# iden3/circom

Measured on NVIDIA H100. Metric: witnesses/s, higher is better.
Workload: dtype u256 (8x u32 limbs, Montgomery)

## Files before the change

### __graft_entry__.py

```python
from __future__ import annotations

import os
import sys

ROOT = os.path.dirname(os.path.abspath(__file__))
if ROOT not in sys.path:
    sys.path.insert(0, ROOT)


def build() -> None:
    from circom_b200 import build as b
    b.build()
    import circom_b200
    from circom_b200 import native
    from tests.util import build_hostsim
    build_hostsim()
    from oracle import build_ref, build_calcs, c_oracle
    c_oracle.build()
    if build_ref.have_reference():
        build_ref.build_all()
        build_calcs.build()


def smoke() -> None:
    import random
    from circom_b200.circuit import CircuitDesc
    from circom_b200 import circuits as C
    from circom_b200.witness_calculator import builder, R1cs, limbs_to_ints
    from oracle.ir_eval import evaluate
    d = CircuitDesc("bn128")
    d.set_main(C.all_ops(d))
# ... 18 lines not shown
```

### circom_b200/csrc/capi.cu

```cuda
#include <cuda_runtime.h>
#include <dlfcn.h>
#include <emmintrin.h>
#include <nccl.h>

#include <cstdio>
#include <cstdlib>
#include <algorithm>
#include <chrono>
#include <condition_variable>
#include <cstring>
#include <functional>
#include <map>
#include <tuple>
#include <memory>
#include <mutex>
#include <thread>
#include <stdexcept>
#include <string>
#include <vector>

#include "../../include/circom_b200.h"
#include <cub/device/device_radix_sort.cuh>

#include "kernels.cuh"
// ... 248 lines not shown
    if ((rc = upload(&d.input_slot, t.input_slot.data(), t.input_slot.size() * 4))) return rc;
    if ((rc = upload(&d.fn_code, t.fn_code.data(), t.fn_code.size() * 4))) return rc;
    if ((rc = upload(&d.fn_info, t.fn_info.data(), t.fn_info.size() * 4))) return rc;
    if ((rc = upload(&d.call_tab, t.call_tab.data(), t.call_tab.size() * 4))) return rc;
    if ((rc = upload(&d.wloc, t.witness_slot.data(), t.witness_slot.size() * 4))) return rc;
    if ((rc = upload(&d.pk_bit, L.bit_loc.data(), L.bit_loc.size() * 4))) return rc;
    if ((rc = upload(&d.pk_u64, L.u64_loc.data(), L.u64_loc.size() * 4))) return rc;
    if ((rc = upload(&d.pk_full, L.full_loc.data(), L.full_loc.size() * 4))) return rc;
    c->dev[device] = d;
    out = d;
    return CW_OK;
}

template <int PR, bool CALLS, bool BP, int BT, bool FU>
static void launch_tape_k(const TapeDev &tp, cw_batch *b, u32 tiles, u32 th) {
    constexpr u32 smem = FU ? TAPE_ACC_SMEM : 0u;
    static_assert(TAPE_ACC_SMEM * CW_TAPE_LB <= 48u * 1024u, "the widest CTA stays within the default dynamic shared memory");
    tape_exec_kernel<PR, CALLS, BP, BT, FU><<<tiles, th, smem * th, b->stream>>>(tp, b->slots, b->plane, b->bt_log2,
                                                                                b->first_assert_d, b->err_d, b->batch);
}
template <int PR>
static void launch_tape(const TapeDev &tp, cw_batch *b, u32 tiles, u32 th, bool calls, bool bp, bool fused) {
    if (calls) {
        launch_tape_calls(PR, tp, b->slots, b->plane, b->bt_log2, b->first_assert_d, b->err_d, b->batch, tiles, th, bp, fused,
                          b->stream);
    } else if (fused) {
        if (b->bt_log2 == 5) launch_tape_k<PR, false, true, 5, true>(tp, b, tiles, th);
        else launch_tape_k<PR, false, true, -1, true>(tp, b, tiles, th);
    } else if (bp) {
        if (b->bt_log2 == 0) launch_tape_k<PR, false, true, 0, false>(tp, b, tiles, th);
        else if (b->bt_log2 == 5) launch_tape_k<PR, false, true, 5, false>(tp, b, tiles, th);
        else launch_tape_k<PR, false, true, -1, false>(tp, b, tiles, th);
    } else {
        if (b->bt_log2 == 0) launch_tape_k<PR, false, false, 0, false>(tp, b, tiles, th);
// ... 1956 lines not shown
```

### circom_b200/csrc/flatten.cpp

```cpp
#include <algorithm>
#include <bitset>
#include <cstdio>
#include <cstdlib>
#include <cstring>
#include <functional>
#include <stdexcept>
#include <unordered_map>

#include "../../include/circom_b200.h"
#include "tape.h"

namespace cw {

uint64_t fnv1a(const char *s, size_t n) {
    uint64_t h = 0xCBF29CE484222325ULL;
    for (size_t i = 0; i < n; ++i) {
        h ^= (uint64_t)(int64_t)(signed char)s[i];
        h *= 0x100000001B3ULL;
    }
    return h;
}

namespace {

// ... 1330 lines not shown
            if (!is_assert && !live[n_pre + i]) continue;
            live[n_pre + i] = 1;
            if (o[0] == 45) {
                uint32_t n = pcalls[o[1] + 1];
                for (uint32_t k = 0; k < n; ++k) {
                    uint32_t a = pcalls[o[1] + 2 + k];
                    if (!(a & OPERAND_CONST)) live[a] = 1;
                }
                continue;
            }
            for (int k = 1; k <= 3; ++k) {
                if (k == 3 && c_is_immediate(o[0])) break;
                if (o[k] != NO_SLOT && !(o[k] & OPERAND_CONST)) live[o[k]] = 1;
            }
        }
        constexpr uint32_t FUSE_MAX = 24;
        enum { FR_READER, FR_POSITION, FR_SIZE, FR_CHAIN, FR_N };
        uint64_t refused[FR_N] = {}, refused_op[64] = {};
        std::vector<uint8_t> fusedf(n_prov, 0);
        std::vector<uint32_t> kid_a(n_prov, NO_SLOT), kid_b(n_prov, NO_SLOT);
        {
            std::vector<uint32_t> uses(n_pre + n_prov, 0), cons(n_pre + n_prov, NO_SLOT);
            std::vector<uint8_t> cons_pos(n_pre + n_prov, 0);
            for (size_t i = 0; i < n_prov; ++i) {
                if (!live[n_pre + i]) continue;
                const uint32_t *o = &pops[i * 4];
                if (o[0] == 45) {
                    uint32_t n = pcalls[o[1] + 1];
                    for (uint32_t k = 0; k < n; ++k) {
                        uint32_t x = pcalls[o[1] + 2 + k];
                        if (!(x & OPERAND_CONST)) uses[x] += 2;
                    }
// ... 13 lines not shown
            auto candidate = [&](uint32_t slot, size_t reader, int pos) -> bool {
                if (!fuse_on || slot == NO_SLOT || (slot & OPERAND_CONST) || slot < n_pre) return false;
                const size_t c = slot - n_pre;
                const uint32_t opc = pops[c * 4];
                if (uses[slot] != 1 || cons[slot] != reader || cons_pos[slot] != pos || claimed[slot] >= 0) return false;
                if (is_assert_op(opc) || opc == 45 || opc == 47 || opc == CW_OP_COPY) return false;
                if (opc == CW_OP_INV || opc == CW_OP_POW) return false;
                return true;
            };
            auto decide = [&](size_t i) {
                const uint32_t *o = &pops[i * 4];
                uint32_t ka = candidate(o[1], i, 1) ? o[1] - n_pre : NO_SLOT;
                uint32_t kb = candidate(o[2], i, 2) ? o[2] - n_pre : NO_SLOT;
                if (ka != NO_SLOT && kb != NO_SLOT) {
                    uint32_t deep = need[ka] >= need[kb] ? ka : kb, other = deep == ka ? kb : ka;
                    if (need[other] > 1 || gsize[ka] + gsize[kb] + 1 > FUSE_MAX) {
                        uint32_t drop = gsize[ka] >= gsize[kb] ? kb : ka;
                        if (need[other] > 1) drop = other;
                        ++refused[need[other] > 1 ? FR_CHAIN : FR_SIZE];
                        if (drop == ka) ka = NO_SLOT; else kb = NO_SLOT;
                    }
                }
                if (ka != NO_SLOT && kb == NO_SLOT && gsize[ka] + 1 > FUSE_MAX) { ka = NO_SLOT; ++refused[FR_SIZE]; }
                if (kb != NO_SLOT && ka == NO_SLOT && gsize[kb] + 1 > FUSE_MAX) { kb = NO_SLOT; ++refused[FR_SIZE]; }
                kid_a[i] = ka;
                kid_b[i] = kb;
                uint32_t sz = 1;
                uint8_t nd = 1;
                if (ka != NO_SLOT && kb != NO_SLOT) {
                    sz += gsize[ka] + gsize[kb];
                    nd = (uint8_t)std::max<int>(std::max(need[ka], need[kb]), std::min(need[ka], need[kb]) + 1);
                } else if (ka != NO_SLOT) { sz += gsize[ka]; nd = need[ka]; }
                else if (kb != NO_SLOT) { sz += gsize[kb]; nd = need[kb]; }
                gsize[i] = sz;
// ... 33 lines not shown
                const uint32_t opc = pops[i * 4];
                if (opc == 45 || opc == 47 || opc == CW_OP_INV || opc == CW_OP_POW) continue;
                regroup(i);
                decide(i);
            }
            const char *cenv = getenv("CW_FUSION_CENSUS");
            if (fuse_on && cenv && atoi(cenv)) {
                for (size_t c = 0; c < n_prov; ++c) {
                    const uint32_t s = n_pre + (uint32_t)c, opc = pops[c * 4];
                    if (!live[s] || fusedf[c] || uses[s] != 1 || claimed[s] >= 0 || is_assert_op(opc)) continue;
                    const uint32_t rd = pops[(size_t)cons[s] * 4];
                    if (rd == 45 || rd == 47 || rd == CW_OP_INV || rd == CW_OP_POW) ++refused[FR_READER];
                    else if (cons_pos[s] == 3) ++refused[FR_POSITION];
                    else if (!candidate(s, cons[s], cons_pos[s])) ++refused_op[opc & 63u];
                }
                fprintf(stderr, "fusion census: single-reader values kept in the store: reader INV/POW %llu, operand c %llu, "
                        "FUSE_MAX %llu, chain rule %llu, producer opcode",
                        (unsigned long long)refused[FR_READER], (unsigned long long)refused[FR_POSITION],
                        (unsigned long long)refused[FR_SIZE], (unsigned long long)refused[FR_CHAIN]);
                for (int k = 0; k < 64; ++k)
                    if (refused_op[k]) fprintf(stderr, " %d:%llu", k, (unsigned long long)refused_op[k]);
                fprintf(stderr, "\n");
            }
        }
        std::vector<uint32_t> glevel(n_pre + n_prov, 0);
        std::vector<uint64_t> gsig(n_prov, 0);
        uint32_t max_level = 0;
        size_t n_roots = 0;
        {
            std::vector<uint32_t> ext(n_prov, 0);
            for (size_t i = 0; i < n_prov; ++i) {
                if (!live[n_pre + i]) continue;
                const uint32_t *o = &pops[i * 4];
                uint32_t e = 0;
// ... 46 lines not shown
        }
        for (size_t r = 0; r < order.size(); ++r) {
            uint32_t p = n_pre + order[r];
            if (claimed[p] >= 0) remap[p] = (uint32_t)claimed[p];
            else if (!is_assert_op(pops[(size_t)order[r] * 4])) remap[p] = next_tmp++;
            if (pops[(size_t)order[r] * 4] == 45) {
                const uint32_t *ct = &pcalls[pops[(size_t)order[r] * 4 + 1]];
                const uint32_t *ex = ct + 2 + ct[1];
                for (uint32_t k = 0; k < ex[0]; ++k) {
                    const uint32_t s = ex[1 + k];
                    if (!live[s]) continue;
                    remap[s] = claimed[s] >= 0 ? (uint32_t)claimed[s] : next_tmp++;
                }
            }
        }
        if (next_tmp >= DST_ACC) throw std::runtime_error("circuit too large for the packed tape word (2^24 slots)");
        T.ops.clear();
        T.ops.reserve(n_live_ops(live, n_pre, n_prov) * 4);
        T.items.clear();
        T.items.reserve(n_roots + 1);
        T.level_start.assign(max_level + 1, 0);
        T.n_mul_ops = 0;
        uint32_t prev_level = 0;
        const bool narrow_on = !(flags & (CW_FLAG_NO_NARROW | CW_FLAG_NO_PEEPHOLE));
        auto opd_bits = [&](uint32_t o) -> uint32_t {
            if (o == NO_SLOT) return 0;
            if (o & OPERAND_CONST) return (uint32_t)u256_bitlen(consts[o & 0x7FFFFFFFu]);
            return o < slot_bits.size() ? slot_bits[o] : 256u;
        };
        auto const_amount = [&](uint32_t o, uint32_t &k) {
            if (o == NO_SLOT || !(o & OPERAND_CONST)) return false;
// ... 50 lines not shown
                }
                const uint32_t *ex = &pcalls[o[1] + 2 + n];
                T.call_tab.push_back(ex[0]);
                for (uint32_t k = 0; k < ex[0]; ++k) T.call_tab.push_back(live[ex[1 + k]] ? remap[ex[1 + k]] : NO_SLOT);
                return;
            }
            for (int k = 1; k <= 3; ++k) {
                if (k == 3 && c_is_immediate(o[0])) d[k] = o[k];
                else if (o[k] == NO_SLOT) d[k] = OPERAND_CONST;
                else if (o[k] & OPERAND_CONST) d[k] = o[k];
                else if (k == 1 && acc_a >= 0) d[k] = OPERAND_ACC | (uint32_t)acc_a;
                else if (k == 2 && acc_b >= 0) d[k] = OPERAND_ACC | (uint32_t)acc_b;
                else d[k] = remap[o[k]];
            }
        };
        std::function<void(uint32_t, int)> emit_sub = [&](uint32_t i, int target) {
            const uint32_t ka = kid_a[i], kb = kid_b[i];
            int acc_a = -1, acc_b = -1;
            if (ka != NO_SLOT && kb != NO_SLOT) {
                const bool a_first = subtree_need(ka, kid_a, kid_b) >= subtree_need(kb, kid_a, kid_b);
                if (a_first) { emit_sub(ka, target); emit_sub(kb, target ^ 1); }
                else { emit_sub(kb, target); emit_sub(ka, target ^ 1); }
                acc_a = a_first ? target : (target ^ 1);
                acc_b = a_first ? (target ^ 1) : target;
            } else if (ka != NO_SLOT) { emit_sub(ka, target); acc_a = target; }
            else if (kb != NO_SLOT) { emit_sub(kb, target); acc_b = target; }
            uint32_t d[4];
            word(i, DST_ACC + (uint32_t)target, acc_a, acc_b, d);
            census(i, d[0] & 0xFFu);
            T.ops.insert(T.ops.end(), d, d + 4);
            if (pops[(size_t)i * 4] == CW_OP_MUL) ++T.n_mul_ops;
        };
        for (size_t r = 0; r < order.size(); ++r) {
            const uint32_t i = order[r];
            const uint32_t *o = &pops[(size_t)i * 4];
            const uint32_t lvl = glevel[n_pre + i];
            const uint32_t dst = is_assert_op(o[0]) ? 0u : remap[n_pre + i];
            const uint32_t ka = kid_a[i], kb = kid_b[i];
            const bool single = ka == NO_SLOT && kb == NO_SLOT;
            uint32_t d[4];
            if (single) {
                word(i, dst, -1, -1, d);
                if (o[0] == DOP_BITS && !(flags & CW_FLAG_NO_PEEPHOLE) && lvl == prev_level && !T.ops.empty() &&
// ... 1 lines not shown
                    uint32_t *p = &T.ops[T.ops.size() - 4];
                    if ((p[0] & 0xFFu) == DOP_BITS && p[1] == d[1] && ((p[3] >> 16) & 0xFFu) == 1u && ((d[3] >> 16) & 0xFFu) == 1u) {
                        uint32_t cnt = (p[3] >> 24) + 1u, pk = p[3] & 0xFFFFu, pdst = p[0] >> 8;
                        if (cnt < 32u && (d[3] & 0xFFFFu) == pk + cnt && dst == pdst + cnt) {
                            p[3] += 1u << 24;
                            continue;
                        }
                    }
                }
                if (o[0] != 45) census(i, d[0] & 0xFFu);
                T.items.push_back((uint32_t)(T.ops.size() / 4));
                T.ops.insert(T.ops.end(), d, d + 4);
            } else {
                T.items.push_back((uint32_t)(T.ops.size() / 4));
                int acc_a = -1, acc_b = -1;
                if (ka != NO_SLOT && kb != NO_SLOT) {
                    const bool a_first = subtree_need(ka, kid_a, kid_b) >= subtree_need(kb, kid_a, kid_b);
                    if (a_first) { emit_sub(ka, 0); emit_sub(kb, 1); }
                    else { emit_sub(kb, 0); emit_sub(ka, 1); }
                    acc_a = a_first ? 0 : 1;
                    acc_b = a_first ? 1 : 0;
                } else if (ka != NO_SLOT) { emit_sub(ka, 0); acc_a = 0; }
                else { emit_sub(kb, 0); acc_b = 0; }
                word(i, dst, acc_a, acc_b, d);
                census(i, d[0] & 0xFFu);
                T.ops.insert(T.ops.end(), d, d + 4);
            }
            prev_level = lvl;
            if (o[0] == CW_OP_MUL) ++T.n_mul_ops;
            T.level_start[lvl]++;
        }
        T.items.push_back((uint32_t)(T.ops.size() / 4));
        {
            std::vector<uint32_t> ls(max_level + 1, 0);
            uint32_t acc = 0;
            uint64_t widest = 0;
            for (uint32_t l = 1; l <= max_level; ++l) {
                ls[l - 1] = acc;
// ... 22 lines not shown
                const uint32_t *o = &T.ops[i * 4];
                if ((o[0] & 0xFFu) == DOP_BITS && (o[3] >> 24) && !(o[1] & OPERAND_CONST) && code[o[1]] != NO_SLOT) ok = false;
            }
            for (uint32_t i = 0; ok && i < M.n_in + 1; ++i)
                if (code[remap[i]] != NO_SLOT) ok = false;
            if (next_tmp >= OPERAND_BIT) ok = false;
            if (ok) {
                newid.resize(next_tmp);
                uint32_t nw = 0;
                for (uint32_t s = 0; s < next_tmp; ++s) newid[s] = code[s] == NO_SLOT ? nw++ : code[s];
                uint32_t word = 0;
                for (size_t i = 0; i < n_ops; ++i) {
                    uint32_t *o = &T.ops[i * 4];
                    const uint32_t opc = o[0] & 0xFFu;
                    if (opc == DOP_BITS && (o[3] >> 24)) o[0] = opc | (word++ << 8);
                    else if (!is_assert_op(opc) && (o[0] >> 8) < DST_ACC) o[0] = opc | (newid[o[0] >> 8] << 8);
                    if (opc == 45) continue;
                    for (int k = 1; k <= 3; ++k) {
                        if (k == 3 && c_is_immediate(opc)) break;
                        if (!(o[k] & (OPERAND_CONST | OPERAND_ACC))) o[k] = newid[o[k]];
                    }
                }
                for (size_t i = 0; i < T.call_tab.size();) {
                    const uint32_t n = T.call_tab[i + 1], nx = T.call_tab[i + 2 + n];
                    for (uint32_t k = 0; k < n + 1 + nx; ++k) {
                        if (k == n) continue;
                        uint32_t &e = T.call_tab[i + 2 + k];
                        if (!(e & OPERAND_CONST)) e = newid[e];
                    }
                    i += 3 + n + nx;
                }
// ... 22 lines not shown
                        continue;
                    }
                    for (int k = 1; k <= 3; ++k) {
                        if (k == 3 && c_is_immediate(opc)) break;
                        if (is_tmp(o[k])) last[o[k]] = (uint32_t)l;
                    }
                }
            std::vector<std::vector<uint32_t>> release(n_lv + 1);
            std::vector<uint32_t> free_ids;
            uint32_t next_phys = n_resident;
            for (size_t l = 0; l < n_lv; ++l) {
                for (uint32_t p : release[l]) free_ids.push_back(p);
                for (uint32_t i = T.items[T.level_start[l]]; i < T.items[T.level_start[l + 1]]; ++i) {
                    uint32_t *o = &T.ops[(size_t)i * 4];
                    const uint32_t opc = o[0] & 0xFFu, d = o[0] >> 8;
                    if (is_assert_op(opc) || d >= DST_ACC) continue;
                    const uint32_t run = opc == DOP_BITS ? (o[3] >> 24) + 1u : 1u;
                    if (run > 1) {
                        if (T.n_bitwords || d < n_resident) continue;
                        for (uint32_t j = 0; j < run; ++j) phys[d + j] = next_phys++;
                        continue;
                    }
                    auto alloc = [&](uint32_t d) {
                        if (d < n_resident) return;
                        uint32_t p;
                        if (!free_ids.empty()) { p = free_ids.back(); free_ids.pop_back(); }
                        else p = next_phys++;
                        phys[d] = p;
                        release[std::min<size_t>(std::max<size_t>(last[d], l) + 1, n_lv)].push_back(p);
                    };
                    alloc(d);
                    if (opc == 45) {
                        const uint32_t *ex = &T.call_tab[o[1] + 2 + T.call_tab[o[1] + 1]];
                        for (uint32_t k = 0; k < ex[0]; ++k)
                            if (ex[1 + k] != NO_SLOT) alloc(ex[1 + k]);
                    }
                }
            }
            auto map = [&](uint32_t o) { return is_tmp(o) ? phys[o] : o; };
            for (size_t i = 0; i < n_ops; ++i) {
                uint32_t *o = &T.ops[i * 4];
                const uint32_t opc = o[0] & 0xFFu;
                if (!is_assert_op(opc) && !(opc == DOP_BITS && (o[3] >> 24) && T.n_bitwords) && (o[0] >> 8) >= n_resident &&
                    (o[0] >> 8) < DST_ACC)
                    o[0] = opc | (phys[o[0] >> 8] << 8);
                if (opc == 45) continue;
                for (int k = 1; k <= 3; ++k) {
                    if (k == 3 && c_is_immediate(opc)) break;
                    o[k] = map(o[k]);
                }
            }
            for (size_t i = 0; i < T.call_tab.size();) {
                const uint32_t n = T.call_tab[i + 1], nx = T.call_tab[i + 2 + n];
                for (uint32_t k = 0; k < n + 1 + nx; ++k)
                    if (k != n) T.call_tab[i + 2 + k] = map(T.call_tab[i + 2 + k]);
                i += 3 + n + nx;
            }
            next_tmp = next_phys;
        }
        T.n_resident = n_resident;
        {
            T.n_slot_operands = 0;
            T.n_values = 0;
            T.n_stored = 0;
            const size_t n_ops = T.ops.size() / 4;
            for (size_t i = 0; i < n_ops; ++i) {
                const uint32_t *o = &T.ops[i * 4];
                const uint32_t opc = o[0] & 0xFFu;
                if (!is_assert_op(opc)) T.n_values += opc == DOP_BITS ? (o[3] >> 24) + 1u : 1u;
                if (!is_assert_op(opc) && (o[0] >> 8) < DST_ACC) ++T.n_stored;
                if (opc == 45) {
                    const uint32_t *ex = &T.call_tab[o[1] + 2 + T.call_tab[o[1] + 1]];
                    for (uint32_t k = 0; k < ex[0]; ++k)
                        if (ex[1 + k] != NO_SLOT) { ++T.n_values; ++T.n_stored; }
                    continue;
                }
                for (int k = 1; k <= 3; ++k) {
                    if (k == 3 && c_is_immediate(opc)) break;
                    if (!(o[k] & (OPERAND_CONST | OPERAND_BIT | OPERAND_ACC))) ++T.n_slot_operands;
                }
            }
        }
        T.witness_slot.resize(W);
        for (uint64_t i = 0; i < W; ++i) T.witness_slot[i] = newid.empty() ? (uint32_t)i : newid[i];
        T.input_slot.resize(M.n_in);
// ... 64 lines not shown
    template <class T> void vec(std::vector<T> &v) {
        uint64_t n;
        pod(n);
        if (n > (uint64_t)(end - p) / sizeof(T)) throw std::runtime_error("lowered-circuit blob: bad length");
        v.resize(n);
        if (n) raw(v.data(), n * sizeof(T));
    }
    void str(std::string &s) {
        uint64_t n;
        pod(n);
        if (n > (uint64_t)(end - p)) throw std::runtime_error("lowered-circuit blob: bad length");
        s.assign((const char *)p, n);
        p += n;
    }
};
constexpr uint32_t BLOB_VERSION = 7;
}

void serialize_tape(const Tape &t, std::vector<uint8_t> &out) {
    BlobW w{out};
    w.raw("CB2T", 4);
    w.pod<uint32_t>(BLOB_VERSION);
    w.pod<int32_t>(t.F.prime_id);
    w.pod(t.flags);
    const uint64_t nums[] = {t.n_signals, t.n_witness, t.n_inputs, t.n_outputs, t.n_components, t.n_ir_ops, t.n_mul_ops,
                             t.n_conv_ops, t.max_level_width, t.n_asserts, t.slot_census[0], t.slot_census[1],
                             t.slot_census[2], t.slot_census[3], t.n_slot_operands, t.n_values, t.n_resident, t.n_pre,
                             t.n_slots, t.n_bitwords, t.n_stored};
    w.pod<uint64_t>(sizeof(nums) / 8);
    w.raw(nums, sizeof(nums));
    w.vec(t.ops); w.vec(t.items); w.vec(t.level_start); w.vec(t.consts); w.vec(t.dat_consts); w.vec(t.witness_slot); w.vec(t.input_slot);
    w.vec(t.pk_bit_wire); w.vec(t.pk_u64_wire); w.vec(t.pk_full_wire); w.vec(t.wit_class); w.vec(t.wit_bits);
    w.vec(t.fn_code); w.vec(t.fn_info); w.vec(t.call_tab); w.vec(t.witness2signal);
    w.raw(t.width_census, sizeof(t.width_census));
    w.pod<uint64_t>(t.inputs.size());
    for (const InputInfo &in : t.inputs) {
        w.str(in.name);
        w.pod(in.hash); w.pod(in.signal_id); w.pod(in.size);
    }
    w.vec(t.hashmap);
    const R1csData &r = t.r1cs;
    w.pod<int32_t>(r.prime_id);
    w.pod(r.n_wires); w.pod(r.n_constraints);
// ... 3 lines not shown

void deserialize_tape(const uint8_t *data, size_t len, Tape &t) {
    BlobR r{data, data + len};
    char magic[4];
    r.raw(magic, 4);
    uint32_t ver;
    r.pod(ver);
    if (memcmp(magic, "CB2T", 4) || ver != BLOB_VERSION) throw std::runtime_error("lowered-circuit blob: bad magic / version");
    int32_t prime;
    r.pod(prime);
    if (prime < 0 || prime >= CW_N_PRIMES) throw std::runtime_error("lowered-circuit blob: unknown prime");
    t.F = make_field(prime);
    r.pod(t.flags);
    uint64_t n_nums;
    r.pod(n_nums);
    uint64_t nums[21];
    if (n_nums != 21) throw std::runtime_error("lowered-circuit blob: layout mismatch");
    r.raw(nums, sizeof(nums));
    t.n_signals = nums[0]; t.n_witness = nums[1]; t.n_inputs = nums[2]; t.n_outputs = nums[3]; t.n_components = nums[4];
    t.n_ir_ops = nums[5]; t.n_mul_ops = nums[6]; t.n_conv_ops = nums[7]; t.max_level_width = nums[8]; t.n_asserts = nums[9];
    for (int k = 0; k < 4; ++k) t.slot_census[k] = nums[10 + k];
    t.n_slot_operands = nums[14]; t.n_values = nums[15]; t.n_resident = (uint32_t)nums[16]; t.n_pre = (uint32_t)nums[17];
    t.n_slots = (uint32_t)nums[18]; t.n_bitwords = (uint32_t)nums[19]; t.n_stored = nums[20];
    r.vec(t.ops); r.vec(t.items); r.vec(t.level_start); r.vec(t.consts); r.vec(t.dat_consts); r.vec(t.witness_slot); r.vec(t.input_slot);
    r.vec(t.pk_bit_wire); r.vec(t.pk_u64_wire); r.vec(t.pk_full_wire); r.vec(t.wit_class); r.vec(t.wit_bits);
    r.vec(t.fn_code); r.vec(t.fn_info); r.vec(t.call_tab); r.vec(t.witness2signal);
    r.raw(t.width_census, sizeof(t.width_census));
    uint64_t n_in;
    r.pod(n_in);
    if (n_in > len) throw std::runtime_error("lowered-circuit blob: bad length");
    t.inputs.resize(n_in);
    for (InputInfo &in : t.inputs) {
        r.str(in.name);
        r.pod(in.hash); r.pod(in.signal_id); r.pod(in.size);
    }
    r.vec(t.hashmap);
    R1csData &R = t.r1cs;
    int32_t rp;
    r.pod(rp);
    R.prime_id = rp;
    r.pod(R.n_wires); r.pod(R.n_constraints);
    r.vec(R.row_ptr); r.vec(R.col); r.vec(R.coef); r.vec(R.dict);
    r.pod(R.n_pub_out); r.pod(R.n_pub_in); r.pod(R.n_prv_in);
    if (t.ops.size() % 4 || t.level_start.empty() || t.items.empty() || t.level_start.back() != t.items.size() - 1 ||
        t.items.back() != t.ops.size() / 4 ||
        t.witness_slot.size() != t.n_witness || t.input_slot.size() != t.n_inputs || t.wit_class.size() != t.n_witness || t.wit_bits.size() != t.n_witness ||
        t.witness2signal.size() != t.n_witness || R.row_ptr.size() != 3 * R.n_constraints + 1 || R.col.size() != R.coef.size() ||
        (R.row_ptr.size() && R.row_ptr.back() != R.col.size()) || t.hashmap.empty())
        throw std::runtime_error("lowered-circuit blob: inconsistent");
}

}
```

### circom_b200/csrc/kernels.cuh

```cuda
#pragma once
#include <cuda_runtime.h>
#include <stdint.h>

#include "fr_device.cuh"
#include "ntt.cuh"
#include "r1cs_small.h"

namespace cw {

constexpr int N_PRIMES_DEV = 8;
__constant__ FrParams c_fr[N_PRIMES_DEV];
#define CW_FR(PRIME, rt) c_fr[(PRIME) >= 0 ? (PRIME) : (int)(rt)]

__device__ __forceinline__ void ldg256(u32 *v, const void *p) {
    asm volatile("ld.global.v4.b32 {%0,%1,%2,%3}, [%8];\n\t"
                 "ld.global.v4.b32 {%4,%5,%6,%7}, [%8+16];"
                 : "=r"(v[0]), "=r"(v[1]), "=r"(v[2]), "=r"(v[3]), "=r"(v[4]), "=r"(v[5]), "=r"(v[6]), "=r"(v[7])
                 : "l"(p)
                 : "memory");
}
__device__ __forceinline__ void ldg256_nc(u32 *v, const void *p) {
    asm("ld.global.nc.v4.b32 {%0,%1,%2,%3}, [%8];\n\t"
        "ld.global.nc.v4.b32 {%4,%5,%6,%7}, [%8+16];"
        : "=r"(v[0]), "=r"(v[1]), "=r"(v[2]), "=r"(v[3]), "=r"(v[4]), "=r"(v[5]), "=r"(v[6]), "=r"(v[7])
// ... 23 lines not shown
    if (bt_log2 == 0) {
        stg256(tile_base + ((size_t)slot << 1), v);
        return;
    }
    size_t i = ((size_t)slot << (bt_log2 + 1)) + inst;
    tile_base[i] = make_uint4(v[0], v[1], v[2], v[3]);
    tile_base[i + ((size_t)1 << bt_log2)] = make_uint4(v[4], v[5], v[6], v[7]);
}
__device__ __forceinline__ void load_const(u32 *v, const uint4 *__restrict__ consts, u32 idx) {
    uint4 lo = __ldg(&consts[2 * (size_t)idx]);
    uint4 hi = __ldg(&consts[2 * (size_t)idx + 1]);
    v[0] = lo.x; v[1] = lo.y; v[2] = lo.z; v[3] = lo.w;
    v[4] = hi.x; v[5] = hi.y; v[6] = hi.z; v[7] = hi.w;
}
constexpr u32 OPD_CONST = 0x80000000u, OPD_BIT = 0x20000000u, OPD_ACC = 0x10000000u, OPD_SLOT = 0x00FFFFFFu, OPD_BITPOS = 0x1FFFFFFFu;
constexpr u32 DST_ACC_DEV = 0x00FFFFFEu;

__device__ __forceinline__ u32 load_plane_bit(const u32 *__restrict__ plane_base, u32 pos, u32 bt_log2, u32 li) {
    return (plane_base[((size_t)(pos >> 5) << bt_log2) + li] >> (pos & 31u)) & 1u;
}

__device__ __forceinline__ void load_slot_low(u32 *v, const uint4 *__restrict__ tile_base, u32 slot, u32 bt_log2, u32 inst) {
    uint4 lo;
    if (bt_log2 == 0) {
        asm volatile("ld.global.v4.b32 {%0,%1,%2,%3}, [%4];" : "=r"(lo.x), "=r"(lo.y), "=r"(lo.z), "=r"(lo.w)
                     : "l"(tile_base + ((size_t)slot << 1)) : "memory");
    } else {
        lo = tile_base[((size_t)slot << (bt_log2 + 1)) + inst];
    }
    v[0] = lo.x; v[1] = lo.y; v[2] = lo.z; v[3] = lo.w;
    v[4] = v[5] = v[6] = v[7] = 0;
// ... 113 lines not shown
        if (d == 0xFFFFFFFFu) continue;
        if (k + 1 >= ret_cnt) { e = 2; continue; }
        u32 v[8];
        vm_result(v, regs, ret_base + k + 1, narrow);
        store_slot(v, base, d, bt_log2, li);
    }
    *err = e;
}

#ifndef CW_TAPE_LB
#define CW_TAPE_LB 512
#endif
#ifndef CW_TAPE_MINB
#define CW_TAPE_MINB 2
#endif
constexpr u32 TAPE_ACC_SMEM = 2 * 8 * 4;
template <int PRIME, bool HAS_CALLS, bool BP, int BT, bool FUSED>
__global__ void __launch_bounds__(CW_TAPE_LB, CW_TAPE_MINB)
    tape_exec_kernel(TapeDev tp, uint4 *__restrict__ slots, u32 *__restrict__ plane, u32 bt_log2_arg,
                     u32 *__restrict__ first_assert, int *__restrict__ err, u32 batch) {
    const FrParams &P = CW_FR(PRIME, tp.prime);
    const u32 bt_log2 = BT >= 0 ? (u32)BT : bt_log2_arg;
    constexpr bool COOP = BT == 0 && !HAS_CALLS && !BP;
    const u32 tile = blockIdx.x;
    const u32 bt_mask = (1u << bt_log2) - 1;
    uint4 *base = slots + (((size_t)tile * tp.n_slots) << (bt_log2 + 1));
    u32 *plane_base = BP ? plane + (((size_t)tile * tp.n_bitwords) << bt_log2) : nullptr;
    extern __shared__ uint4 tape_smem[];
    u32 *const acc = reinterpret_cast<u32 *>(tape_smem) + threadIdx.x;
    u32 lb = tp.level_start[0];
    u32 le = tp.n_levels ? tp.level_start[1] : lb;
// ... 45 lines not shown
                        run_n = run;
                        run_bits = (u32)window;
                    } else {
                        for (u32 j = 0; j < run; ++j) {
                            r[0] = (u32)(window >> j) & 1u;
                            store_slot(r, base, dst + j, bt_log2, li);
                        }
                    }
                    has_value = false;
                } else r[0] = (u32)window & (m >= 32u ? 0xFFFFFFFFu : ((1u << m) - 1u));
            } else {
                u32 a[8], b[8];
                const bool half = opcode >= OP_NARROW_HALF;
                if (FUSED && !(opw.y & OPD_CONST) && (opw.y & OPD_ACC)) {
#pragma unroll
                    for (int i = 0; i < 8; ++i) a[i] = acc[(8 * (opw.y & 1u) + i) * blockDim.x];
                } else load_operand<BP>(a, opw.y, base, plane_base, tp.consts, bt_log2, li, half);
                if (FUSED && !(opw.z & OPD_CONST) && (opw.z & OPD_ACC)) {
#pragma unroll
                    for (int i = 0; i < 8; ++i) b[i] = acc[(8 * (opw.z & 1u) + i) * blockDim.x];
                } else load_operand<BP>(b, opw.z, base, plane_base, tp.consts, bt_log2, li, half);
                if (opcode == OP_SELECT) {
                    u32 c[8];
                    load_operand<BP>(c, opw.w, base, plane_base, tp.consts, bt_log2, li);
                    bool t = !u256_is_zero(c);
#pragma unroll
                    for (int i = 0; i < 8; ++i) r[i] = t ? a[i] : b[i];
                } else if (opcode == OP_ASSERT_EQ || opcode == OP_ASSERT || opcode == OP_ASSERT_BOOL ||
                           opcode == OP_ASSERT_FITS) {
                    bool ok = opcode == OP_ASSERT_EQ     ? u256_eq(a, b)
                              : opcode == OP_ASSERT      ? !u256_is_zero(a)
                              : opcode == OP_ASSERT_BOOL ? (u256_is_zero(a) || u256_eq(a, b))
                                                         : (u256_bitlen_dev(a) <= b[0]);
                    if (!ok && inst < batch) atomicMin(&first_assert[inst], opw.w);
                    has_value = false;
                } else if (opcode == OP_INV || opcode == OP_POW) {
                    has_value = false;
                } else {
                    int e = 0;
                    fr_exec_t<false>(opcode, r, a, b, opw.w, P, e);
                    if (e && inst < batch) err[inst] = 1;
                }
            }
            if (has_value) {
                if (FUSED && dst >= DST_ACC_DEV) {
#pragma unroll
                    for (int i = 0; i < 8; ++i) acc[(8 * (dst & 1u) + i) * blockDim.x] = r[i];
                } else store_slot(r, base, dst, bt_log2, li);
            }
            }
            }
            if (COOP) {
                unsigned pending = __ballot_sync(0xFFFFFFFFu, run_n != 0u);
                const u32 lane = threadIdx.x & 31u;
                while (pending) {
                    const int src = __ffs(pending) - 1;
                    pending &= pending - 1u;
                    const u32 d = __shfl_sync(0xFFFFFFFFu, run_dst, src);
                    const u32 cnt = __shfl_sync(0xFFFFFFFFu, run_n, src);
                    const u32 bits = __shfl_sync(0xFFFFFFFFu, run_bits, src);
                    if (lane < cnt) {
                        u32 r[8] = {(bits >> lane) & 1u, 0u, 0u, 0u, 0u, 0u, 0u, 0u};
// ... 533 lines not shown
```

### circom_b200/csrc/tape.h

```cpp
#pragma once
#include <cstdint>
#include <string>
#include <vector>

#include "u256.h"
#include "r1cs_small.h"

namespace cw {

constexpr uint32_t OPERAND_CONST = 0x80000000u;
constexpr uint32_t OPERAND_SLOT_MASK = 0x00FFFFFFu;
constexpr uint32_t OPERAND_BIT = 0x20000000u, OPERAND_BITPOS_MASK = 0x1FFFFFFFu;
constexpr uint32_t OPERAND_ACC = 0x10000000u, DST_ACC = 0x00FFFFFEu;
constexpr uint32_t WSLOT_MONT = 0x80000000u;
constexpr uint32_t NO_SLOT = 0xFFFFFFFFu;

struct InputInfo {
    std::string name;
    uint64_t hash;
    uint64_t signal_id;
    uint64_t size;
};

struct HashEntry {
    uint64_t hash, signalid, signalsize;
};

struct R1csData {
// ... 12 lines not shown

struct Tape {
    FieldParams F;
    uint32_t flags = 0;
    uint64_t n_signals = 0, n_witness = 0, n_inputs = 0, n_outputs = 0, n_components = 0;
    uint64_t n_ir_ops = 0, n_mul_ops = 0, n_conv_ops = 0, max_level_width = 0, n_asserts = 0;
    uint64_t slot_census[4] = {0, 0, 0, 0};
    uint64_t width_census[64 * 4] = {};
    uint64_t n_slot_operands = 0;
    uint64_t n_stored = 0;
    uint64_t n_values = 0;
    uint32_t n_resident = 0;
    uint32_t n_pre = 0;
    uint32_t n_slots = 0;
    uint32_t n_bitwords = 0;
    std::vector<uint32_t> ops;
    std::vector<uint32_t> items;
    std::vector<uint32_t> level_start;
    std::vector<U256> consts;
    std::vector<U256> dat_consts;
    std::vector<uint32_t> witness_slot;
    std::vector<uint32_t> input_slot;
    std::vector<uint32_t> pk_bit_wire, pk_u64_wire, pk_full_wire;
    std::vector<uint8_t> wit_class;
    std::vector<uint16_t> wit_bits;
    std::vector<uint32_t> fn_code, fn_info, call_tab;
    std::vector<uint64_t> witness2signal;
    std::vector<InputInfo> inputs;
    std::vector<HashEntry> hashmap;
    R1csData r1cs;
// ... 69 lines not shown
```

### circom_b200/native.py

```python
from __future__ import annotations

import ctypes
import os
from ctypes import POINTER, c_char_p, c_float, c_int, c_int32, c_int64, c_size_t, c_uint8, c_uint32, c_uint64, c_void_p

from . import build as _build

CW_OK, CW_EINVAL, CW_EIO, CW_EFORMAT, CW_ECUDA, CW_ENOTFOUND, CW_ESTATE, CW_ENODEV = 0, -1, -2, -3, -4, -5, -6, -7
CW_FLAG_NO_ASSERTS, CW_FLAG_HOST_ONLY, CW_FLAG_O0, CW_FLAG_NO_PEEPHOLE, CW_FLAG_BITPLANE, CW_FLAG_REUSE = 1, 2, 4, 8, 16, 32
CW_FLAG_COMPACT = CW_FLAG_BITPLANE | CW_FLAG_REUSE
CW_FLAG_FUSE = 64
CW_FLAG_NO_NARROW = 128
CW_NTT_FORWARD, CW_NTT_INVERSE, CW_NTT_COSET = 0, 1, 2


class CwError(RuntimeError):
    def __init__(self, code: int, msg: str):
        super().__init__("circom_b200 error %d: %s" % (code, msg))
        self.code = code


class CwStats(ctypes.Structure):
    _fields_ = [(n, c_uint64) for n in (
        "n_signals", "n_witness", "n_inputs", "n_outputs", "n_components", "n_constants", "n_ir_ops",
        "n_tape_ops", "n_slots", "n_levels", "n_constraints", "n_nnz", "n_mul_ops", "n_conv_ops",
        "max_level_width", "n_slot_operands", "n_bitwords", "n_resident_slots", "n_items", "n_stored", "n_values")]
# ... 116 lines not shown
```

### circom_b200/witness_calculator.py

```python
from __future__ import annotations

import ctypes
import os
from typing import Dict, Iterable, List, Optional, Sequence, Union

import numpy as np

from . import native
from .circuit import CircuitDesc
from .native import CwError, CwStats, check, lib


def fnv_hash(s: str) -> int:
    h = 0xCBF29CE484222325
    for ch in s:
        h ^= ord(ch)
        h = (h * 0x100000001B3) & 0xFFFFFFFFFFFFFFFF
    return h


def _flat(a) -> list:
    out = []

    def rec(x):
# ... 88 lines not shown
            libc.madvise(ctypes.c_void_p(raw.ctypes.data + off), ctypes.c_size_t(n & ~((2 << 20) - 1)), 14)
        except (OSError, AttributeError):
            pass
    return raw[off:off + n].view(dtype).reshape(shape)


class Circuit:

    def __init__(self, src: Union[CircuitDesc, bytes, str], sanity_check: bool = True, host_only: bool = False,
                 o0: bool = False, flags: int = 0, compact: Optional[bool] = None, fuse: bool = False,
                 symbols: bool = False):
        if compact is None:
            compact = os.environ.get("CW_COMPACT", "1") != "0" and not (flags & native.CW_FLAG_COMPACT)
        flags |= int(os.environ.get("CW_FLAGS_EXTRA", "0"))
        if fuse:
            flags |= native.CW_FLAG_FUSE
        flags |= (0 if sanity_check else native.CW_FLAG_NO_ASSERTS) | (native.CW_FLAG_HOST_ONLY if host_only else 0) | \
            (native.CW_FLAG_O0 if o0 else 0) | (native.CW_FLAG_COMPACT if compact else 0)
        self.flags = flags
        self._h = ctypes.c_void_p()
        if isinstance(src, CircuitDesc):
            src = src.to_bytes(symbols=symbols)
        if isinstance(src, (bytes, bytearray)):
            buf = bytes(src)
            check(lib.cw_circuit_load_mem(buf, len(buf), flags, ctypes.byref(self._h)))
        else:
            check(lib.cw_circuit_load(str(src).encode(), flags, ctypes.byref(self._h)))
        self._init_from_handle()

    @classmethod
    def from_handle(cls, handle: ctypes.c_void_p, flags: int = 0) -> "Circuit":
# ... 430 lines not shown
```

### include/circom_b200.h

```cpp
#ifndef CIRCOM_B200_H
#define CIRCOM_B200_H

#include <stddef.h>
#include <stdint.h>

#ifdef __cplusplus
extern "C" {
#endif

#define CW_OK 0
#define CW_EINVAL (-1)
#define CW_EIO (-2)
#define CW_EFORMAT (-3)
#define CW_ECUDA (-4)
#define CW_ENOTFOUND (-5)
#define CW_ESTATE (-6)
#define CW_ENODEV (-7)

#define CW_PRIME_BN128 0
#define CW_PRIME_BLS12381 1
#define CW_PRIME_GRUMPKIN 2
#define CW_PRIME_PALLAS 3
#define CW_PRIME_VESTA 4
#define CW_PRIME_SECQ256R1 5
#define CW_PRIME_BLS12377 6
#define CW_PRIME_GOLDILOCKS 7

#define CW_FLAG_NO_ASSERTS 1u
#define CW_FLAG_HOST_ONLY 2u
#define CW_FLAG_NO_PEEPHOLE 8u
#define CW_FLAG_BITPLANE 16u
#define CW_FLAG_REUSE 32u
#define CW_FLAG_FUSE 64u
#define CW_FLAG_NO_NARROW 128u
#define CW_FLAG_COMPACT (CW_FLAG_BITPLANE | CW_FLAG_REUSE)
#define CW_FLAG_O0 4u

enum cw_op {
    CW_OP_NOP = 0, CW_OP_MUL = 1, CW_OP_DIV = 2, CW_OP_ADD = 3, CW_OP_SUB = 4, CW_OP_POW = 5,
    CW_OP_IDIV = 6, CW_OP_MOD = 7, CW_OP_SHL = 8, CW_OP_SHR = 9, CW_OP_LEQ = 10, CW_OP_GEQ = 11,
    CW_OP_LT = 12, CW_OP_GT = 13, CW_OP_EQ = 14, CW_OP_NEQ = 15, CW_OP_LOR = 16, CW_OP_LAND = 17,
    CW_OP_LNOT = 18, CW_OP_BOR = 19, CW_OP_BAND = 20, CW_OP_BXOR = 21, CW_OP_BNOT = 22,
    CW_OP_NEG = 23, CW_OP_COPY = 24, CW_OP_SELECT = 25, CW_OP_ASSERT = 26, CW_OP_ASSERT_EQ = 27,
    CW_OP_INV = 28
};

typedef struct cw_circuit cw_circuit;
typedef struct cw_batch cw_batch;
// ... 144 lines not shown
```

Baseline: 202,700.

## Generalize fused-expression accumulators from two to up to eight per work item

Widens the fused expression-tree lowering so a work item can hold up to eight accumulators in shared memory instead of two. Deeper subtrees can then be fused rather than spilled back to the slot store. The fusion limits become tunable, with a deep-fuse flag raising the defaults to 4 accumulators and 32 ops, and the Python builder sets it whenever fuse is requested. Dynamic shared memory is now sized from the tape's accumulator count, which raises per-CTA shared memory and may lower occupancy. The blob format gains an n_acc field and a validation pass.

```diff
diff --git a/__graft_entry__.py b/__graft_entry__.py
--- a/__graft_entry__.py
+++ b/__graft_entry__.py
@@ -15,6 +15,8 @@
     from circom_b200 import native
     from tests.util import build_hostsim
     build_hostsim()
+    from tests.accsim import build_accsim
+    build_accsim()
     from oracle import build_ref, build_calcs, c_oracle
     c_oracle.build()
     if build_ref.have_reference():
diff --git a/circom_b200/csrc/capi.cu b/circom_b200/csrc/capi.cu
--- a/circom_b200/csrc/capi.cu
+++ b/circom_b200/csrc/capi.cu
@@ -286,10 +286,11 @@
 
 template <int PR, bool CALLS, bool BP, int BT, bool FU>
 static void launch_tape_k(const TapeDev &tp, cw_batch *b, u32 tiles, u32 th) {
-    constexpr u32 smem = FU ? TAPE_ACC_SMEM : 0u;
-    static_assert(TAPE_ACC_SMEM * CW_TAPE_LB <= 48u * 1024u, "the widest CTA stays within the default dynamic shared memory");
-    tape_exec_kernel<PR, CALLS, BP, BT, FU><<<tiles, th, smem * th, b->stream>>>(tp, b->slots, b->plane, b->bt_log2,
-                                                                                b->first_assert_d, b->err_d, b->batch);
+    const size_t smem = FU ? (size_t)TAPE_ACC_SMEM * b->c->tape.n_acc * th : 0u;
+    if (smem > 48u * 1024u)
+        cudaFuncSetAttribute(tape_exec_kernel<PR, CALLS, BP, BT, FU>, cudaFuncAttributeMaxDynamicSharedMemorySize, (int)smem);
+    tape_exec_kernel<PR, CALLS, BP, BT, FU><<<tiles, th, smem, b->stream>>>(tp, b->slots, b->plane, b->bt_log2,
+                                                                           b->first_assert_d, b->err_d, b->batch);
 }
 template <int PR>
 static void launch_tape(const TapeDev &tp, cw_batch *b, u32 tiles, u32 th, bool calls, bool bp, bool fused) {
diff --git a/circom_b200/csrc/flatten.cpp b/circom_b200/csrc/flatten.cpp
--- a/circom_b200/csrc/flatten.cpp
+++ b/circom_b200/csrc/flatten.cpp
@@ -1368,8 +1368,16 @@
                 if (o[k] != NO_SLOT && !(o[k] & OPERAND_CONST)) live[o[k]] = 1;
             }
         }
-        constexpr uint32_t FUSE_MAX = 24;
-        enum { FR_READER, FR_POSITION, FR_SIZE, FR_CHAIN, FR_N };
+        auto env_knob = [](const char *name, uint32_t dflt, uint32_t lo, uint32_t hi) {
+            const char *s = getenv(name);
+            if (!s || !*s) return dflt;
+            const long v = atol(s);
+            return (uint32_t)std::min<long>(std::max<long>(v, lo), hi);
+        };
+        const bool deep = (flags & CW_FLAG_FUSE_DEEP) != 0;
+        const uint32_t FUSE_ACC = env_knob("CW_FUSE_ACC", deep ? 4 : 2, 1, ACC_MAX);
+        const uint32_t FUSE_MAX = env_knob("CW_FUSE_MAX", deep ? 32 : 24, 1, 256);
+        enum { FR_READER, FR_POSITION, FR_SIZE, FR_ACC, FR_N };
         uint64_t refused[FR_N] = {}, refused_op[64] = {};
         std::vector<uint8_t> fusedf(n_prov, 0);
         std::vector<uint32_t> kid_a(n_prov, NO_SLOT), kid_b(n_prov, NO_SLOT);
@@ -1413,10 +1421,11 @@
                 uint32_t kb = candidate(o[2], i, 2) ? o[2] - n_pre : NO_SLOT;
                 if (ka != NO_SLOT && kb != NO_SLOT) {
                     uint32_t deep = need[ka] >= need[kb] ? ka : kb, other = deep == ka ? kb : ka;
-                    if (need[other] > 1 || gsize[ka] + gsize[kb] + 1 > FUSE_MAX) {
+                    const bool too_many = std::max<uint32_t>(need[deep], need[other] + 1u) > FUSE_ACC;
+                    if (too_many || gsize[ka] + gsize[kb] + 1 > FUSE_MAX) {
                         uint32_t drop = gsize[ka] >= gsize[kb] ? kb : ka;
-                        if (need[other] > 1) drop = other;
-                        ++refused[need[other] > 1 ? FR_CHAIN : FR_SIZE];
+                        if (too_many) drop = other;
+                        ++refused[too_many ? FR_ACC : FR_SIZE];
                         if (drop == ka) ka = NO_SLOT; else kb = NO_SLOT;
                     }
                 }
@@ -1480,10 +1489,10 @@
                     else if (cons_pos[s] == 3) ++refused[FR_POSITION];
                     else if (!candidate(s, cons[s], cons_pos[s])) ++refused_op[opc & 63u];
                 }
-                fprintf(stderr, "fusion census: single-reader values kept in the store: reader INV/POW %llu, operand c %llu, "
-                        "FUSE_MAX %llu, chain rule %llu, producer opcode",
-                        (unsigned long long)refused[FR_READER], (unsigned long long)refused[FR_POSITION],
-                        (unsigned long long)refused[FR_SIZE], (unsigned long long)refused[FR_CHAIN]);
+                fprintf(stderr, "fusion census (FUSE_ACC %u, FUSE_MAX %u): single-reader values kept in the store: reader "
+                        "INV/POW %llu, operand c %llu, FUSE_MAX %llu, needs more than FUSE_ACC accumulators %llu, producer opcode",
+                        FUSE_ACC, FUSE_MAX, (unsigned long long)refused[FR_READER], (unsigned long long)refused[FR_POSITION],
+                        (unsigned long long)refused[FR_SIZE], (unsigned long long)refused[FR_ACC]);
                 for (int k = 0; k < 64; ++k)
                     if (refused_op[k]) fprintf(stderr, " %d:%llu", k, (unsigned long long)refused_op[k]);
                 fprintf(stderr, "\n");
@@ -1560,7 +1569,7 @@
                 }
             }
         }
-        if (next_tmp >= DST_ACC) throw std::runtime_error("circuit too large for the packed tape word (2^24 slots)");
+        if (next_tmp >= DST_ACC_LO) throw std::runtime_error("circuit too large for the packed tape word (2^24 slots)");
         T.ops.clear();
         T.ops.reserve(n_live_ops(live, n_pre, n_prov) * 4);
         T.items.clear();
@@ -1641,19 +1650,26 @@
                 else d[k] = remap[o[k]];
             }
         };
-        std::function<void(uint32_t, int)> emit_sub = [&](uint32_t i, int target) {
+        T.n_acc = 0;
+        std::function<void(uint32_t, int)> emit_sub;
+        auto emit_kids = [&](uint32_t i, int target, int &acc_a, int &acc_b) {
             const uint32_t ka = kid_a[i], kb = kid_b[i];
-            int acc_a = -1, acc_b = -1;
             if (ka != NO_SLOT && kb != NO_SLOT) {
                 const bool a_first = subtree_need(ka, kid_a, kid_b) >= subtree_need(kb, kid_a, kid_b);
-                if (a_first) { emit_sub(ka, target); emit_sub(kb, target ^ 1); }
-                else { emit_sub(kb, target); emit_sub(ka, target ^ 1); }
-                acc_a = a_first ? target : (target ^ 1);
-                acc_b = a_first ? (target ^ 1) : target;
+                if (a_first) { emit_sub(ka, target); emit_sub(kb, target + 1); }
+                else { emit_sub(kb, target); emit_sub(ka, target + 1); }
+                acc_a = a_first ? target : target + 1;
+                acc_b = a_first ? target + 1 : target;
             } else if (ka != NO_SLOT) { emit_sub(ka, target); acc_a = target; }
             else if (kb != NO_SLOT) { emit_sub(kb, target); acc_b = target; }
+        };
+        emit_sub = [&](uint32_t i, int target) {
+            if ((uint32_t)target >= ACC_MAX) throw std::runtime_error("lowering: fused work item needs too many accumulators");
+            T.n_acc = std::max(T.n_acc, (uint32_t)target + 1);
+            int acc_a = -1, acc_b = -1;
+            emit_kids(i, target, acc_a, acc_b);
             uint32_t d[4];
-            word(i, DST_ACC + (uint32_t)target, acc_a, acc_b, d);
+            word(i, acc_dst((uint32_t)target), acc_a, acc_b, d);
             census(i, d[0] & 0xFFu);
             T.ops.insert(T.ops.end(), d, d + 4);
             if (pops[(size_t)i * 4] == CW_OP_MUL) ++T.n_mul_ops;
@@ -1685,14 +1701,7 @@
             } else {
                 T.items.push_back((uint32_t)(T.ops.size() / 4));
                 int acc_a = -1, acc_b = -1;
-                if (ka != NO_SLOT && kb != NO_SLOT) {
-                    const bool a_first = subtree_need(ka, kid_a, kid_b) >= subtree_need(kb, kid_a, kid_b);
-                    if (a_first) { emit_sub(ka, 0); emit_sub(kb, 1); }
-                    else { emit_sub(kb, 0); emit_sub(ka, 1); }
-                    acc_a = a_first ? 0 : 1;
-                    acc_b = a_first ? 1 : 0;
-                } else if (ka != NO_SLOT) { emit_sub(ka, 0); acc_a = 0; }
-                else { emit_sub(kb, 0); acc_b = 0; }
+                emit_kids(i, 0, acc_a, acc_b);
                 word(i, dst, acc_a, acc_b, d);
                 census(i, d[0] & 0xFFu);
                 T.ops.insert(T.ops.end(), d, d + 4);
@@ -1745,7 +1754,7 @@
                     uint32_t *o = &T.ops[i * 4];
                     const uint32_t opc = o[0] & 0xFFu;
                     if (opc == DOP_BITS && (o[3] >> 24)) o[0] = opc | (word++ << 8);
-                    else if (!is_assert_op(opc) && (o[0] >> 8) < DST_ACC) o[0] = opc | (newid[o[0] >> 8] << 8);
+                    else if (!is_assert_op(opc) && (o[0] >> 8) < DST_ACC_LO) o[0] = opc | (newid[o[0] >> 8] << 8);
                     if (opc == 45) continue;
                     for (int k = 1; k <= 3; ++k) {
                         if (k == 3 && c_is_immediate(opc)) break;
@@ -1798,7 +1807,7 @@
                 for (uint32_t i = T.items[T.level_start[l]]; i < T.items[T.level_start[l + 1]]; ++i) {
                     uint32_t *o = &T.ops[(size_t)i * 4];
                     const uint32_t opc = o[0] & 0xFFu, d = o[0] >> 8;
-                    if (is_assert_op(opc) || d >= DST_ACC) continue;
+                    if (is_assert_op(opc) || d >= DST_ACC_LO) continue;
                     const uint32_t run = opc == DOP_BITS ? (o[3] >> 24) + 1u : 1u;
                     if (run > 1) {
                         if (T.n_bitwords || d < n_resident) continue;
@@ -1826,7 +1835,7 @@
                 uint32_t *o = &T.ops[i * 4];
                 const uint32_t opc = o[0] & 0xFFu;
                 if (!is_assert_op(opc) && !(opc == DOP_BITS && (o[3] >> 24) && T.n_bitwords) && (o[0] >> 8) >= n_resident &&
-                    (o[0] >> 8) < DST_ACC)
+                    (o[0] >> 8) < DST_ACC_LO)
                     o[0] = opc | (phys[o[0] >> 8] << 8);
                 if (opc == 45) continue;
                 for (int k = 1; k <= 3; ++k) {
@@ -1852,7 +1861,7 @@
                 const uint32_t *o = &T.ops[i * 4];
                 const uint32_t opc = o[0] & 0xFFu;
                 if (!is_assert_op(opc)) T.n_values += opc == DOP_BITS ? (o[3] >> 24) + 1u : 1u;
-                if (!is_assert_op(opc) && (o[0] >> 8) < DST_ACC) ++T.n_stored;
+                if (!is_assert_op(opc) && (o[0] >> 8) < DST_ACC_LO) ++T.n_stored;
                 if (opc == 45) {
                     const uint32_t *ex = &T.call_tab[o[1] + 2 + T.call_tab[o[1] + 1]];
                     for (uint32_t k = 0; k < ex[0]; ++k)
@@ -1947,7 +1956,7 @@
         p += n;
     }
 };
-constexpr uint32_t BLOB_VERSION = 7;
+constexpr uint32_t BLOB_VERSION = 8;
 }
 
 void serialize_tape(const Tape &t, std::vector<uint8_t> &out) {
@@ -1959,7 +1968,7 @@
     const uint64_t nums[] = {t.n_signals, t.n_witness, t.n_inputs, t.n_outputs, t.n_components, t.n_ir_ops, t.n_mul_ops,
                              t.n_conv_ops, t.max_level_width, t.n_asserts, t.slot_census[0], t.slot_census[1],
                              t.slot_census[2], t.slot_census[3], t.n_slot_operands, t.n_values, t.n_resident, t.n_pre,
-                             t.n_slots, t.n_bitwords, t.n_stored};
+                             t.n_slots, t.n_bitwords, t.n_stored, t.n_acc};
     w.pod<uint64_t>(sizeof(nums) / 8);
     w.raw(nums, sizeof(nums));
     w.vec(t.ops); w.vec(t.items); w.vec(t.level_start); w.vec(t.consts); w.vec(t.dat_consts); w.vec(t.witness_slot); w.vec(t.input_slot);
@@ -1993,14 +2002,16 @@
     r.pod(t.flags);
     uint64_t n_nums;
     r.pod(n_nums);
-    uint64_t nums[21];
-    if (n_nums != 21) throw std::runtime_error("lowered-circuit blob: layout mismatch");
+    uint64_t nums[22];
+    if (n_nums != 22) throw std::runtime_error("lowered-circuit blob: layout mismatch");
     r.raw(nums, sizeof(nums));
     t.n_signals = nums[0]; t.n_witness = nums[1]; t.n_inputs = nums[2]; t.n_outputs = nums[3]; t.n_components = nums[4];
     t.n_ir_ops = nums[5]; t.n_mul_ops = nums[6]; t.n_conv_ops = nums[7]; t.max_level_width = nums[8]; t.n_asserts = nums[9];
     for (int k = 0; k < 4; ++k) t.slot_census[k] = nums[10 + k];
     t.n_slot_operands = nums[14]; t.n_values = nums[15]; t.n_resident = (uint32_t)nums[16]; t.n_pre = (uint32_t)nums[17];
     t.n_slots = (uint32_t)nums[18]; t.n_bitwords = (uint32_t)nums[19]; t.n_stored = nums[20];
+    if (nums[21] > ACC_MAX) throw std::runtime_error("lowered-circuit blob: too many accumulators");
+    t.n_acc = (uint32_t)nums[21];
     r.vec(t.ops); r.vec(t.items); r.vec(t.level_start); r.vec(t.consts); r.vec(t.dat_consts); r.vec(t.witness_slot); r.vec(t.input_slot);
     r.vec(t.pk_bit_wire); r.vec(t.pk_u64_wire); r.vec(t.pk_full_wire); r.vec(t.wit_class); r.vec(t.wit_bits);
     r.vec(t.fn_code); r.vec(t.fn_info); r.vec(t.call_tab); r.vec(t.witness2signal);
@@ -2027,6 +2038,14 @@
         t.witness2signal.size() != t.n_witness || R.row_ptr.size() != 3 * R.n_constraints + 1 || R.col.size() != R.coef.size() ||
         (R.row_ptr.size() && R.row_ptr.back() != R.col.size()) || t.hashmap.empty())
         throw std::runtime_error("lowered-circuit blob: inconsistent");
+    for (size_t i = 0; i < t.ops.size(); i += 4) {
+        const uint32_t opc = t.ops[i] & 0xFFu, dst = t.ops[i] >> 8;
+        bool bad = opc != 45 && !is_assert_op(opc) && dst >= DST_ACC_LO && acc_of_dst(dst) >= t.n_acc;
+        for (int k = 1; k <= 2; ++k)
+            bad |= opc != 45 && !(t.ops[i + k] & (OPERAND_CONST | OPERAND_BIT)) && (t.ops[i + k] & OPERAND_ACC) &&
+                   (t.ops[i + k] & ACC_MASK) >= t.n_acc;
+        if (bad) throw std::runtime_error("lowered-circuit blob: accumulator beyond n_acc");
+    }
 }
 
 }
diff --git a/circom_b200/csrc/kernels.cuh b/circom_b200/csrc/kernels.cuh
--- a/circom_b200/csrc/kernels.cuh
+++ b/circom_b200/csrc/kernels.cuh
@@ -61,7 +61,7 @@
     v[4] = hi.x; v[5] = hi.y; v[6] = hi.z; v[7] = hi.w;
 }
 constexpr u32 OPD_CONST = 0x80000000u, OPD_BIT = 0x20000000u, OPD_ACC = 0x10000000u, OPD_SLOT = 0x00FFFFFFu, OPD_BITPOS = 0x1FFFFFFFu;
-constexpr u32 DST_ACC_DEV = 0x00FFFFFEu;
+constexpr u32 DST_ACC_DEV = 0x00FFFFF8u, ACC_MASK_DEV = 7u, ACC_DST_SWIZZLE_DEV = 6u;
 
 __device__ __forceinline__ u32 load_plane_bit(const u32 *__restrict__ plane_base, u32 pos, u32 bt_log2, u32 li) {
     return (plane_base[((size_t)(pos >> 5) << bt_log2) + li] >> (pos & 31u)) & 1u;
@@ -205,7 +205,7 @@
 #ifndef CW_TAPE_MINB
 #define CW_TAPE_MINB 2
 #endif
-constexpr u32 TAPE_ACC_SMEM = 2 * 8 * 4;
+constexpr u32 TAPE_ACC_SMEM = 8 * 4;
 template <int PRIME, bool HAS_CALLS, bool BP, int BT, bool FUSED>
 __global__ void __launch_bounds__(CW_TAPE_LB, CW_TAPE_MINB)
     tape_exec_kernel(TapeDev tp, uint4 *__restrict__ slots, u32 *__restrict__ plane, u32 bt_log2_arg,
@@ -281,11 +281,11 @@
                 const bool half = opcode >= OP_NARROW_HALF;
                 if (FUSED && !(opw.y & OPD_CONST) && (opw.y & OPD_ACC)) {
 #pragma unroll
-                    for (int i = 0; i < 8; ++i) a[i] = acc[(8 * (opw.y & 1u) + i) * blockDim.x];
+                    for (int i = 0; i < 8; ++i) a[i] = acc[(8 * (opw.y & ACC_MASK_DEV) + i) * blockDim.x];
                 } else load_operand<BP>(a, opw.y, base, plane_base, tp.consts, bt_log2, li, half);
                 if (FUSED && !(opw.z & OPD_CONST) && (opw.z & OPD_ACC)) {
 #pragma unroll
-                    for (int i = 0; i < 8; ++i) b[i] = acc[(8 * (opw.z & 1u) + i) * blockDim.x];
+                    for (int i = 0; i < 8; ++i) b[i] = acc[(8 * (opw.z & ACC_MASK_DEV) + i) * blockDim.x];
                 } else load_operand<BP>(b, opw.z, base, plane_base, tp.consts, bt_log2, li, half);
                 if (opcode == OP_SELECT) {
                     u32 c[8];
@@ -312,7 +312,7 @@
             if (has_value) {
                 if (FUSED && dst >= DST_ACC_DEV) {
 #pragma unroll
-                    for (int i = 0; i < 8; ++i) acc[(8 * (dst & 1u) + i) * blockDim.x] = r[i];
+                    for (int i = 0; i < 8; ++i) acc[(8 * ((dst ^ ACC_DST_SWIZZLE_DEV) & ACC_MASK_DEV) + i) * blockDim.x] = r[i];
                 } else store_slot(r, base, dst, bt_log2, li);
             }
             }
diff --git a/circom_b200/csrc/tape.h b/circom_b200/csrc/tape.h
--- a/circom_b200/csrc/tape.h
+++ b/circom_b200/csrc/tape.h
@@ -11,7 +11,10 @@
 constexpr uint32_t OPERAND_CONST = 0x80000000u;
 constexpr uint32_t OPERAND_SLOT_MASK = 0x00FFFFFFu;
 constexpr uint32_t OPERAND_BIT = 0x20000000u, OPERAND_BITPOS_MASK = 0x1FFFFFFFu;
-constexpr uint32_t OPERAND_ACC = 0x10000000u, DST_ACC = 0x00FFFFFEu;
+constexpr uint32_t OPERAND_ACC = 0x10000000u, DST_ACC = 0x00FFFFFEu, DST_ACC_LO = 0x00FFFFF8u, ACC_MASK = 7u, ACC_MAX = 8u;
+constexpr uint32_t ACC_DST_SWIZZLE = 6u;
+inline uint32_t acc_dst(uint32_t k) { return DST_ACC_LO | (k ^ ACC_DST_SWIZZLE); }
+inline uint32_t acc_of_dst(uint32_t dst) { return (dst ^ ACC_DST_SWIZZLE) & ACC_MASK; }
 constexpr uint32_t WSLOT_MONT = 0x80000000u;
 constexpr uint32_t NO_SLOT = 0xFFFFFFFFu;
 
@@ -54,6 +57,7 @@
     uint32_t n_pre = 0;
     uint32_t n_slots = 0;
     uint32_t n_bitwords = 0;
+    uint32_t n_acc = 0;
     std::vector<uint32_t> ops;
     std::vector<uint32_t> items;
     std::vector<uint32_t> level_start;
diff --git a/circom_b200/native.py b/circom_b200/native.py
--- a/circom_b200/native.py
+++ b/circom_b200/native.py
@@ -10,6 +10,7 @@
 CW_FLAG_NO_ASSERTS, CW_FLAG_HOST_ONLY, CW_FLAG_O0, CW_FLAG_NO_PEEPHOLE, CW_FLAG_BITPLANE, CW_FLAG_REUSE = 1, 2, 4, 8, 16, 32
 CW_FLAG_COMPACT = CW_FLAG_BITPLANE | CW_FLAG_REUSE
 CW_FLAG_FUSE = 64
+CW_FLAG_FUSE_DEEP = 256
 CW_FLAG_NO_NARROW = 128
 CW_NTT_FORWARD, CW_NTT_INVERSE, CW_NTT_COSET = 0, 1, 2
 
diff --git a/circom_b200/witness_calculator.py b/circom_b200/witness_calculator.py
--- a/circom_b200/witness_calculator.py
+++ b/circom_b200/witness_calculator.py
@@ -126,7 +126,7 @@
             compact = os.environ.get("CW_COMPACT", "1") != "0" and not (flags & native.CW_FLAG_COMPACT)
         flags |= int(os.environ.get("CW_FLAGS_EXTRA", "0"))
         if fuse:
-            flags |= native.CW_FLAG_FUSE
+            flags |= native.CW_FLAG_FUSE | native.CW_FLAG_FUSE_DEEP
         flags |= (0 if sanity_check else native.CW_FLAG_NO_ASSERTS) | (native.CW_FLAG_HOST_ONLY if host_only else 0) | \
             (native.CW_FLAG_O0 if o0 else 0) | (native.CW_FLAG_COMPACT if compact else 0)
         self.flags = flags
diff --git a/include/circom_b200.h b/include/circom_b200.h
--- a/include/circom_b200.h
+++ b/include/circom_b200.h
@@ -32,6 +32,7 @@
 #define CW_FLAG_BITPLANE 16u
 #define CW_FLAG_REUSE 32u
 #define CW_FLAG_FUSE 64u
+#define CW_FLAG_FUSE_DEEP 256u
 #define CW_FLAG_NO_NARROW 128u
 #define CW_FLAG_COMPACT (CW_FLAG_BITPLANE | CW_FLAG_REUSE)
 #define CW_FLAG_O0 4u
```

New measurement: 207,500, median of 6. 1.02x the previous value.
